# nianticlabs/mickey

Measured on AMD Instinct MI355X. Metric: image pairs/sec (540x720), higher is better.
Workload: dtype bf16

## Files before the change

include/mickey_hip_dev.h:

```cpp
#ifndef MICKEY_HIP_DEV_H
#define MICKEY_HIP_DEV_H

#ifdef __cplusplus
extern "C" {
#endif

int mk_gemm_set_tile(int mode);

int mk_attn_set_mode(int mode);

int mk_dev_mfma_sustained(float* scratch, int workgroups, int iters, int zero_operands, void* stream);

#ifdef __cplusplus
}
#endif
#endif
```

mickey_amd/_native.py:

```python
import ctypes
import os

import torch

from . import build as _build

MK_BF16, MK_F16, MK_F32 = 0, 1, 2
ACT_NONE, ACT_RELU, ACT_GELU = 0, 1, 2

_P, _I, _L, _F, _U = ctypes.c_void_p, ctypes.c_int, ctypes.c_longlong, ctypes.c_float, ctypes.c_ulonglong
_CODES = {"p": _P, "i": _I, "l": _L, "f": _F, "u": _U}

SIGNATURES = {
    "mk_version": ("i", ""),
    "mk_last_error": ("s", ""),
    "mk_preprocess_u8": ("i", "pliiipiip"),
    "mk_gemm": ("i", "pipippiiiiiiip"),
    "mk_gemm_grouped": ("i", "pilpilplpiliiiiiiip"),
    "mk_gemm_ls_residual": ("i", "pipipppiiiiip"),
    "mk_gemm_qkv": ("i", "pipippppiiiifip"),
    "mk_gemm_patch_embed": ("i", "pipipppiiiiip"),
    "mk_gemm_ls_residual_ln": ("i", "pipippppipppiiiiip"),
    "mk_gemm_patch_embed_ln": ("i", "pipipppppiiiiip"),
    "mk_cls_token_ln": ("i", "pppppiiiip"),
# ... 61 lines not shown
    "mk_dual_softmax": ("i", "ppppfifppppiiiip"),
    "mk_dual_softmax_split_work_floats": ("l", "iii"),
    "mk_dual_softmax_split": ("i", "ppppfifppppiiiip"),
    "mk_sinkhorn_work_floats": ("l", "iii"),
    "mk_sinkhorn": ("i", "ppppfippppiiiip"),
    "mk_dual_softmax_kf": ("i", "ppppfifppppiiiipip"),
    "mk_dual_softmax_split_kf": ("i", "ppppfifppppiiiipip"),
    "mk_sinkhorn_kf": ("i", "ppppfippppiiiipip"),
    "mk_mutual_nn": ("i", "ppppiiip"),
    "mk_dual_softmax_train_work_floats": ("l", "iiii"),
    "mk_dual_softmax_train": ("i", "ppppfppppppiiiiip"),
    "mk_dual_softmax_bwd_work_floats": ("l", "iiii"),
    "mk_dual_softmax_bwd": ("i", "ppppfpppppppppiiiiip"),
    "mk_exprace_topk_work_bytes": ("l", "iiil"),
    "mk_exprace_topk_state_bytes": ("l", "ii"),
    "mk_exprace_topk": ("i", "ppuupppppiiliip"),
    "mk_counter_add": ("i", "pup"),
    "mk_gather_backproject": ("i", "ppppppppppppiiiiip"),
    "mk_gather_backproject_kf": ("i", "ppppppppppppiiiiipip"),
    "mk_gather_backproject_bwd": ("i", "ppppppppppiiiiip"),
    "mk_ransac_hypotheses": ("i", "pppppuupfppppiiilp"),
    "mk_refine_pose": ("i", "pppppfiipppppppiiiip"),
    "mk_pose_finalize": ("i", "ppppip"),
    "mk_train_ransac_masks": ("i", "pppppuupfiipppiiilp"),
    "mk_reinforce_scatter": ("i", "ppppiiilp"),
    "mk_train_tail_fwd": ("i", "pppppppiiiifiifpppp"),
    "mk_train_tail_bwd": ("i", "pppppppiiiifiifppppppp"),
    "mk_train_aggregate_fwd": ("i", "pppiiififfppppp"),
    "mk_train_aggregate_bwd": ("i", "ppiiipp"),
}

DEV_SIGNATURES = {
    "mk_gemm_set_tile": ("i", "i"),
    "mk_attn_set_mode": ("i", "i"),
    "mk_dev_mfma_sustained": ("i", "piiip"),
}

_lib = None
_missing = set()


class MickeyHipError(RuntimeError):
    pass


def lib_path():
    return os.environ.get("MICKEY_HIP_LIB", _build.lib_path())


def load():
    global _lib
    if _lib is not None:
        return _lib
    path = lib_path()
    if not os.path.exists(path):
        raise MickeyHipError("libmickey_hip.so not found at %s -- build it with `python -m mickey_amd.build` "
                             "(mickey_amd has no CPU/ATen fallback)" % path)
    lib = ctypes.CDLL(path)
    for name, (res, args) in list(SIGNATURES.items()) + list(DEV_SIGNATURES.items()):
        try:
            fn = getattr(lib, name)
        except AttributeError:
            _missing.add(name)
            continue
        fn.restype = ctypes.c_char_p if res == "s" else _CODES[res]
        fn.argtypes = [_CODES[c] for c in args]
# ... 47 lines not shown
```

mickey_amd/csrc/mk_gemm.hip:

```cpp
#include "mk_gemm_common.hpp"

namespace mk {
namespace gemm {
namespace {

template <typename T, int AMODE, int WMF, bool SP = false>
__global__ __launch_bounds__(256, 1) void gemm_kernel(GemmParams p) {
  using V8 = typename Lp<T>::V8;
  constexpr int NWM = 2, NWN = 2;
  constexpr int NW = NWM * NWN, BM = NWM * WMF * 16, BN = NWN * 64;
  constexpr int AJ = BM / 8 / NW, WJ = BN / 8 / NW;
  constexpr int A_BYTES = BM * 128, STAGE_BYTES = (BM + BN) * 128;
  constexpr int NS = WMF == 2 ? 3 : 2;
  constexpr int PIECES = AJ + WJ;
  extern __shared__ __attribute__((aligned(16))) char smem[];

  const int tid = threadIdx.x;
  const int lane = tid & 63;
  const int wave = __builtin_amdgcn_readfirstlane(tid >> 6);
  const int wm = wave / NWN, wn = wave % NWN;
  const int g = blockIdx.y;
  const int ntm = (p.M + BM - 1) / BM, ntn = (p.N + BN - 1) / BN;
  const int nk = p.K / BK;
  const int fr = lane & 15, fg = lane >> 4;
// ... 63 lines not shown
#pragma unroll
        for (int mi = 0; mi < WMF; ++mi)
#pragma unroll
          for (int ni = 0; ni < 4; ++ni) acc[mi][ni] = Lp<T>::mma16(wf[ni], xf[mi], acc[mi][ni]);
      }
    }
  }
  epilogue<T, WMF>(p, acc, m0, n0, wm, wn, lane, g, lnp);
}

template <typename T, int AMODE, int WMF, bool SP = false>
int launch_small(const GemmParams& p, int groups, hipStream_t st) {
  constexpr int BM = 32 * WMF;
  constexpr int LDS = (WMF == 2 ? 3 : 2) * (BM + 128) * 128 + BM * 8;
  static bool attr_done = false;
  if (!attr_done) {
    hipError_t e = hipFuncSetAttribute((const void*)gemm_kernel<T, AMODE, WMF, SP>, hipFuncAttributeMaxDynamicSharedMemorySize, LDS);
    if (e != hipSuccess) {
      mk_set_error("gemm: cannot reserve %d B of LDS: %s", LDS, hipGetErrorString(e));
      return MK_ERR_LAUNCH;
    }
    attr_done = true;
  }
  const int ntm = (p.M + BM - 1) / BM, ntn = (p.N + 127) / 128;
  hipLaunchKernelGGL((gemm_kernel<T, AMODE, WMF, SP>), dim3(ntm * ntn, groups, 1), dim3(256), LDS, st, p);
  MK_CHECK_LAUNCH();
  return MK_OK;
}

int g_num_cus = 0;
int g_band_m = 0;
int g_half_rows = 1;
int g_schedule = 0;

template <int AMODE>
int launch(const GemmParams& p, int groups, int dtype, hipStream_t st) {
  const long long big_tiles = (long long)((p.M + 255) / 256) * ((p.N + 255) / 256) * groups;
  bool big = p.N >= 256 && big_tiles >= 192;
  const long long plmax = p.npass > 1 ? (long long)max(max(p.pl1[0], p.pl1[1]), max(p.pl2[0], p.pl2[1])) / 2 : 0;
  const bool k_ok = p.K >= 2 * BK && (long long)p.M * p.lda + plmax < (1ll << 31) && (long long)p.N * p.ldw < (1ll << 31) &&
                    (AMODE == A_DENSE || bordered_rows(p.M / (p.H * p.Wd), p.H, p.Wd) * (p.C1 > p.C2 ? p.C1 : p.C2) + plmax < (1ll << 31));
  const bool ln_fold = p.ln_stats || p.xh;
  if (dtype == MK_F32) {
    MK_CHECK_ARG(!ln_fold, "gemm: the folded-LayerNorm epilogues exist for 16-bit operands only");
    return launch_f32(p, groups, AMODE, st);
  }
  int sched = g_schedule;
  if (sched == 0) sched = (big && k_ok) ? 7 : 1;
  if (!k_ok) sched = 1;
  if (sched == 7) return launch_pp64(p, groups, dtype, AMODE, st, g_band_m);
  const long long small_tiles = (long long)((p.M + 127) / 128) * ((p.N + 127) / 128) * groups;
  const bool half_rows = g_schedule == 2 || (g_schedule != 1 && g_half_rows && small_tiles < 2 * num_cus() && p.M > 64);
  if (p.npass > 1)
    return half_rows ? launch_small<_Float16, AMODE, 2, true>(p, groups, st) : launch_small<_Float16, AMODE, 4, true>(p, groups, st);
  if (half_rows) return dtype == MK_BF16 ? launch_small<__bf16, AMODE, 2>(p, groups, st) : launch_small<_Float16, AMODE, 2>(p, groups, st);
  return dtype == MK_BF16 ? launch_small<__bf16, AMODE, 4>(p, groups, st) : launch_small<_Float16, AMODE, 4>(p, groups, st);
}

int check_common(const GemmParams& p, int dtype) {
  MK_CHECK_ARG(dtype == MK_BF16 || dtype == MK_F16 || dtype == MK_F32, "gemm: dtype must be MK_BF16, MK_F16 or MK_F32");
  MK_CHECK_ARG(p.M > 0 && p.N > 0 && p.K > 0, "gemm: empty problem M=%d N=%d K=%d", p.M, p.N, p.K);
  const int kt = dtype == MK_F32 ? KT<float> : BK;
  MK_CHECK_ARG(p.K % kt == 0, "gemm: K=%d must be a multiple of %d", p.K, kt);
  MK_CHECK_ARG(p.N % 4 == 0, "gemm: N=%d must be a multiple of 4", p.N);
  MK_CHECK_ARG(p.ldw % 8 == 0 && p.ldw >= p.K, "gemm: ldw=%d must be >= K and a multiple of 8", p.ldw);
  MK_CHECK_ARG(p.A && p.W, "gemm: null operand");
  return MK_OK;
}

}

int num_cus() {
  if (g_num_cus == 0) {
    int dev = 0, n = 0;
    if (hipGetDevice(&dev) != hipSuccess || hipDeviceGetAttribute(&n, hipDeviceAttributeMultiprocessorCount, dev) != hipSuccess || n <= 0)
      n = 256;
    g_num_cus = n;
  }
  return g_num_cus;
}

}
}

using namespace mk;
using namespace mk::gemm;

extern "C" {

int mk_gemm_set_tile(int mode) {
  if (mode >= 400 && mode < 464) {
    g_band_m = mode - 400;
    return MK_OK;
  }
  if (mode >= 464 && mode < 496) {
    g_band_m = -(mode - 464);
    return MK_OK;
  }
  if (mode == 500 || mode == 501) {
    g_half_rows = mode - 500;
    return MK_OK;
  }
  if (mode >= 600 && mode <= 602) {
    g_pp64_persist = mode - 600;
    return MK_OK;
  }
  MK_CHECK_ARG(mode == 0 || mode == 1 || mode == 2 || mode == 7,
               "mk_gemm_set_tile: unknown mode %d (0 automatic, 1 128x128, 2 64x128, 7 8-wave ping-pong)", mode);
  g_schedule = mode;
  return MK_OK;
}

int mk_gemm(const void* A, int lda, const void* W, int ldw, const float* bias, void* out, int ldc, int M, int N, int K,
            int act, int out_is_f32, int dtype, mk_stream_t stream) {
  GemmParams p = {};
  p.A = A; p.W = W; p.M = M; p.N = N; p.K = K; p.lda = lda; p.ldw = ldw;
  p.epi = MK_EPI_STORE; p.act = act; p.bias = bias; p.ldc = ldc;
  if (out_is_f32) p.out_f32 = (float*)out; else p.out_lp = out;
  if (int e = check_common(p, dtype)) return e;
  MK_CHECK_ARG(lda % 8 == 0 && lda >= K && ldc % 4 == 0 && ldc >= N && out, "mk_gemm: bad lda/ldc/out");
  return launch<A_DENSE>(p, 1, dtype, (hipStream_t)stream);
}

int mk_gemm_grouped(const void* A, int lda, long long strideA, const void* W, int ldw, long long strideW, const float* bias,
                    long long strideBias, void* out, int ldc, long long strideOut, int groups, int M, int N, int K, int act,
                    int out_is_f32, int dtype, mk_stream_t stream) {
  GemmParams p = {};
  p.A = A; p.W = W; p.M = M; p.N = N; p.K = K; p.lda = lda; p.ldw = ldw;
  p.strideA_g = strideA; p.strideW_g = strideW; p.strideBias_g = strideBias; p.strideOut_g = strideOut;
  p.epi = MK_EPI_STORE; p.act = act; p.bias = bias; p.ldc = ldc;
  if (out_is_f32) p.out_f32 = (float*)out; else p.out_lp = out;
  if (int e = check_common(p, dtype)) return e;
  MK_CHECK_ARG(groups > 0 && lda % 8 == 0 && lda >= K && ldc % 4 == 0 && ldc >= N && out, "mk_gemm_grouped: bad args");
  return launch<A_DENSE>(p, groups, dtype, (hipStream_t)stream);
}

int mk_gemm_ls_residual(const void* A, int lda, const void* W, int ldw, const float* bias, const float* gamma, float* x,
                        int ldx, int M, int N, int K, int dtype, mk_stream_t stream) {
  GemmParams p = {};
  p.A = A; p.W = W; p.M = M; p.N = N; p.K = K; p.lda = lda; p.ldw = ldw;
  p.epi = MK_EPI_LS_RESIDUAL; p.bias = bias; p.gamma = gamma; p.out_f32 = x; p.ldc = ldx;
  if (int e = check_common(p, dtype)) return e;
  MK_CHECK_ARG(bias && gamma && x && lda % 8 == 0 && lda >= K && ldx % 4 == 0 && ldx >= N, "mk_gemm_ls_residual: bad args");
  return launch<A_DENSE>(p, 1, dtype, (hipStream_t)stream);
// ... 194 lines not shown
```

mickey_amd/csrc/mk_gemm_common.hpp:

```cpp
#pragma once
#include "mk_common.hpp"

namespace mk {
namespace gemm {

constexpr int BK = 64;
template <typename T> constexpr int EPC = 16 / (int)sizeof(T);
template <typename T> constexpr int KT = 128 / (int)sizeof(T);

enum AMode { A_DENSE = 0, A_CONV3 = 1 };

struct GemmParams {
  const void* A;
  const void* A2;
  const void* W;
  int M, N, K, lda, ldw;
  long long strideA_g, strideA2_g, strideW_g;
  int H, Wd, C1, C2;
  int bord_out;
  unsigned pl1[2], pl2[2];
  int npass;
  float acc_scale;
  void* out_lo;
  float plane_scale;
  int* sat_flag;
  int epi;
  int act;
  const float* bias;
  const float* gamma;
  long long strideBias_g;
  float* out_f32;
  void* out_lp;
  int ldc;
  long long strideOut_g;
  const void* resid_lp;
  long long strideResid_g;
  void* q;
  void* k;
  void* vt;
  int ntok, ntok_pad, heads;
  float qscale;
  const float* pos;
  int npatch;
// ... 439 lines not shown
}

template <typename T, int WMF>
__device__ __forceinline__ void epilogue(const GemmParams& p, f32x4 (&acc)[WMF][4], int m0, int n0, int wm, int wn, int lane,
                                         int g, const float2* lnp = nullptr) {
  if (p.xh) {
    if (p.epi == MK_EPI_PATCH) epilogue_impl<T, WMF, MK_EPI_PATCH, MK_ACT_NONE, true, false, true>(p, acc, m0, n0, wm, wn, lane, g);
    else epilogue_impl<T, WMF, MK_EPI_LS_RESIDUAL, MK_ACT_NONE, true, false, true>(p, acc, m0, n0, wm, wn, lane, g);
    return;
  }
  if (p.ln_stats) {
    if (p.epi == MK_EPI_QKV) epilogue_impl<T, WMF, MK_EPI_QKV, MK_ACT_NONE, true, true>(p, acc, m0, n0, wm, wn, lane, g, lnp);
    else if (p.act == MK_ACT_GELU) epilogue_impl<T, WMF, MK_EPI_STORE, MK_ACT_GELU, true, true>(p, acc, m0, n0, wm, wn, lane, g, lnp);
    else epilogue_impl<T, WMF, MK_EPI_STORE, MK_ACT_NONE, true, true>(p, acc, m0, n0, wm, wn, lane, g, lnp);
    return;
  }
  switch (p.epi) {
    case MK_EPI_LS_RESIDUAL: epilogue_impl<T, WMF, MK_EPI_LS_RESIDUAL, MK_ACT_NONE, true>(p, acc, m0, n0, wm, wn, lane, g); break;
    case MK_EPI_QKV: epilogue_impl<T, WMF, MK_EPI_QKV, MK_ACT_NONE, true>(p, acc, m0, n0, wm, wn, lane, g); break;
    case MK_EPI_PATCH: epilogue_impl<T, WMF, MK_EPI_PATCH, MK_ACT_NONE, true>(p, acc, m0, n0, wm, wn, lane, g); break;
    default:
      if (!p.bias) {
        if (p.act == MK_ACT_RELU) epilogue_impl<T, WMF, MK_EPI_STORE, MK_ACT_RELU, false>(p, acc, m0, n0, wm, wn, lane, g);
        else if (p.act == MK_ACT_GELU) epilogue_impl<T, WMF, MK_EPI_STORE, MK_ACT_GELU, false>(p, acc, m0, n0, wm, wn, lane, g);
        else epilogue_impl<T, WMF, MK_EPI_STORE, MK_ACT_NONE, false>(p, acc, m0, n0, wm, wn, lane, g);
      } else {
        if (p.act == MK_ACT_RELU) epilogue_impl<T, WMF, MK_EPI_STORE, MK_ACT_RELU, true>(p, acc, m0, n0, wm, wn, lane, g);
        else if (p.act == MK_ACT_GELU) epilogue_impl<T, WMF, MK_EPI_STORE, MK_ACT_GELU, true>(p, acc, m0, n0, wm, wn, lane, g);
        else epilogue_impl<T, WMF, MK_EPI_STORE, MK_ACT_NONE, true>(p, acc, m0, n0, wm, wn, lane, g);
      }
  }
}

template <typename T, int EPI, int ACT, bool HAS_BIAS, bool LN = false, bool SPLIT = false, bool FIN = false, bool CONV = false>
__device__ __forceinline__ void epilogue_lds_impl(const GemmParams& p, f32x4 (&acc)[8][4], char* wl0, char* wl1, int m0, int n0, int wm,
                                                  int wn, int lane, int g, const float2* lnp = nullptr) {
  using V4 = typename Lp<T>::V4;
  using V8 = typename Lp<T>::V8;
  const int fr = lane & 15, fg = lane >> 4;
  const float* bias = HAS_BIAS ? p.bias + (long long)g * p.strideBias_g : nullptr;
  const int nw = n0 + wn * 64;
  const int mw = m0 + wm * 128;
  int img0 = 0, tok0 = 0;
  if (EPI == MK_EPI_QKV) {
    img0 = mw / p.ntok;
    tok0 = mw - img0 * p.ntok;
  }
  auto img_tok = [&](int r, int& img, int& tok) {
    if (p.ntok >= 128) {
      const int t = tok0 + r;
      const bool wrap = t >= p.ntok;
      img = img0 + (wrap ? 1 : 0);
      tok = wrap ? t - p.ntok : t;
    } else {
      const int m = mw + r;
      img = m / p.ntok;
      tok = m - img * p.ntok;
    }
  };
  f32x4 bv[4], cs[4];
#pragma unroll
  for (int ni = 0; ni < 4; ++ni) {
    const int n = nw + fg * 4 + ni * 16;
    bv[ni] = (HAS_BIAS && n < p.N) ? *(const f32x4*)(bias + n) : f32x4{0.f, 0.f, 0.f, 0.f};
    cs[ni] = (LN && n < p.N) ? *(const f32x4*)(p.ln_colsum + n) : f32x4{0.f, 0.f, 0.f, 0.f};
  }
  float2 prm[8];
#pragma unroll
  for (int mi = 0; mi < 8; ++mi) prm[mi] = LN ? lnp[wm * 128 + mi * 16 + fr] : make_float2(1.f, 0.f);
  const bool lp_out = EPI == MK_EPI_QKV || (EPI == MK_EPI_STORE && !p.out_f32 && !p.out_lo);
  if (lp_out) {
    int which = 0, head = 0;
    if (EPI == MK_EPI_QKV) {
      const int D = p.heads * 64;
      which = nw / D;
      head = (nw - which * D) >> 6;
      if (which == 2) {
#pragma unroll
        for (int mi = 0; mi < 8; ++mi) {
          const int m = mw + mi * 16 + fr;
          if (m >= p.M) continue;
          int img, tok;
          img_tok(mi * 16 + fr, img, tok);
          const long long hb = (long long)img * p.heads + head;
#pragma unroll
          for (int ni = 0; ni < 4; ++ni) {
            const f32x4 v = LN ? acc[mi][ni] * prm[mi].x + (cs[ni] * prm[mi].y + bv[ni]) : acc[mi][ni] + bv[ni];
            T* dst = (T*)p.vt + (hb * 64 + ni * 16 + fg * 4) * p.ntok_pad + vperm(tok);
#pragma unroll
            for (int e = 0; e < 4; ++e) dst[(long long)e * p.ntok_pad] = to_lp<T>(v[e]);
          }
        }
        return;
      }
    }
    const int rr = lane >> 3, c = lane & 7;
    const int n = nw + c * 8;
    const bool bord = CONV && p.bord_out;
    BorderedRow bw;
    if (bord) bw.init(mw + rr, p.H, p.Wd);
#pragma unroll
    for (int h = 0; h < 2; ++h) {
#pragma unroll
      for (int mq = 0; mq < 4; ++mq) {
        const int mi = h * 4 + mq;
        const int r = mi * 16 + fr;
        char* wrow = (mq < 2 ? wl0 : wl1) + ((mq & 1) * 16 + fr) * 128;
        const long long rrow = (CONV && p.resid_lp) ? bordered_row(min(mw + r, p.M - 1), p.H, p.Wd) : 0;
#pragma unroll
        for (int ni = 0; ni < 4; ++ni) {
          f32x4 v = acc[mi][ni];
          if (LN) v = v * prm[mi].x + (cs[ni] * prm[mi].y + bv[ni]);
          else if (HAS_BIAS) v += bv[ni];
          if (EPI == MK_EPI_QKV) {
            if (which == 0) { const float qs = p.qscale; _Pragma("unroll") for (int e = 0; e < 4; ++e) v[e] *= qs; }
          } else {
            if (CONV && p.resid_lp) {
              const int m = mw + r, n2 = nw + fg * 4 + ni * 16;
              if (m < p.M && n2 < p.N) {
                const V4 rs = *(const V4*)((const T*)p.resid_lp + (long long)g * p.strideResid_g + rrow * p.ldc + n2);
#pragma unroll
                for (int e = 0; e < 4; ++e) v[e] += (float)rs[e];
              }
            }
            if (ACT == MK_ACT_RELU) {
#pragma unroll
              for (int e = 0; e < 4; ++e) v[e] = fmaxf(v[e], 0.f);
            } else if (ACT == MK_ACT_GELU) {
              v = gelu_erf4(v);
            }
          }
          V4 o;
#pragma unroll
          for (int e = 0; e < 4; ++e) o[e] = to_lp<T>(v[e]);
          const int cc = ni * 2 + (fg >> 1);
          *(V4*)(wrow + ((cc ^ (fr & 7)) << 4) + (fg & 1) * 8) = o;
        }
      }
#pragma unroll
      for (int i8 = 0; i8 < 8; ++i8) {
        const int it = h * 8 + i8;
        const int r = it * 8 + rr;
        const int m = mw + r;
        const V8 val = *(const V8*)((i8 < 4 ? wl0 : wl1) + ((i8 & 3) * 8 + rr) * 128 + ((c ^ (rr & 7)) << 4));
        const int extra = bord ? bw.extra : 0;
        if (bord) bw.step(8, p.H, p.Wd);
        if (m >= p.M || n >= p.N) continue;
        T* dst;
        if (EPI == MK_EPI_QKV) {
          int img, tok;
          img_tok(r, img, tok);
          dst = (T*)(which == 0 ? p.q : p.k) + (((long long)img * p.heads + head) * p.ntok_pad + tok) * 64 + c * 8;
        } else {
          dst = (T*)p.out_lp + (long long)g * p.strideOut_g + ((long long)m + extra) * p.ldc + n;
        }
        if (n + 8 <= p.N) {
          *(V8*)dst = val;
        } else {
          V4 lo;
#pragma unroll
          for (int e = 0; e < 4; ++e) lo[e] = val[e];
          *(V4*)dst = lo;
        }
      }
    }
  } else {
    const int rr = lane >> 4, c = lane & 15;
    const int n = nw + c * 4;
    f32x4 gm = f32x4{0.f, 0.f, 0.f, 0.f};
    if (EPI == MK_EPI_LS_RESIDUAL && n < p.N) gm = *(const f32x4*)(p.gamma + n);
    f32x4 bvd = f32x4{0.f, 0.f, 0.f, 0.f};
    if (SPLIT && HAS_BIAS && n < p.N) bvd = *(const f32x4*)(bias + n);
    f32x4 xr[2][SPLIT ? 1 : 16];
// ... 116 lines not shown
          x += gm * val;
          if (SPLIT) x -= ((const float*)lnp)[wm * 128 + half * 64 + r];
          if (!SPLIT || fin) {
            if (ok) *(f32x4*)(p.out_f32 + (long long)m * p.ldc + n) = x;
          } else {
            if constexpr (sizeof(T) == 2) emit_row(m, nullptr, nullptr, x, ok, soff_b(half, it));
            else emit_row(m, plane_row(p.xh, half, it) + lane_off_st, plane_row(p.xl, half, it) + lane_off_st, x, ok);
          }
        } else if (EPI == MK_EPI_PATCH) {
          const int mc = ok ? m : 0;
          const int img = mc / p.npatch, tok = mc - img * p.npatch;
          const long long xrow = (long long)img * (p.npatch + 1) + 1 + tok;
          f32x4 x = val;
          if (ok) x += *(const f32x4*)(p.pos + (long long)(1 + tok) * p.N + n);
          if (SPLIT) emit_row(xrow, (T*)p.xh + xrow * p.ldxs + n, (T*)p.xl + xrow * p.ldxs + n, x, ok);
          else if (ok) *(f32x4*)(p.out_f32 + xrow * p.ldc + n) = x;
        } else if (EPI == MK_EPI_STORE && p.out_lo) {
          const float ps = p.plane_scale;
          f16x4 oh, ol;
#pragma unroll
          for (int e = 0; e < 4; ++e) {
            const float sv = sat16(val[e] * ps, p.sat_flag);
            oh[e] = (_Float16)sv;
            ol[e] = (_Float16)(sv - (float)oh[e]);
          }
          const long long o = (long long)g * p.strideOut_g + ((long long)m + extraf) * p.ldc + n;
          *(f16x4*)((_Float16*)p.out_lp + o) = oh;
          *(f16x4*)((_Float16*)p.out_lo + o) = ol;
        } else {
          *(f32x4*)(p.out_f32 + (long long)g * p.strideOut_g + ((long long)m + extraf) * p.ldc + n) = val;
        }
      }
    };
    if (SPLIT && !FIN && EPI == MK_EPI_LS_RESIDUAL) {
      preload(0, 0, 16);
      stageq(0, 0);
      drain(0, 0, 8);
      preload(1, 0, 8);
      stageq(0, 1);
      drain(0, 8, 16);
      preload(1, 8, 16);
      stageq(1, 0);
      drain(1, 0, 8);
      stageq(1, 1);
      drain(1, 8, 16);
    } else {
      preload(0);
      stageq(0, 0);
      drain(0, 0, 8);
      stageq(0, 1);
      preload(1);
      drain(0, 8, 16);
      stageq(1, 0);
      drain(1, 0, 8);
      stageq(1, 1);
      drain(1, 8, 16);
    }
  }
}

template <typename T, int KIND, bool CONV = false, int BN = 256>
__device__ __forceinline__ void epilogue_lds(const GemmParams& p, f32x4 (&acc)[8][4], char* wl0, char* wl1, int m0, int n0, int wm,
                                             int wn, int lane, int g, const float2* lnp = nullptr) {
  if constexpr (KIND == 2 || KIND == 3) {
    const bool interior = m0 + 256 <= p.M && n0 + BN <= p.N;
    if (KIND == 3) {
      if (interior) epilogue_lds_impl<T, MK_EPI_LS_RESIDUAL, MK_ACT_NONE, true, false, true, true>(p, acc, wl0, wl1, m0, n0, wm, wn, lane, g, lnp);
// ... 3 lines not shown
      else epilogue_impl<T, 8, MK_EPI_PATCH, MK_ACT_NONE, true, false, true>(p, acc, m0, n0, wm, wn, lane, g);
    } else {
      if (interior) epilogue_lds_impl<T, MK_EPI_LS_RESIDUAL, MK_ACT_NONE, true, false, true, false>(p, acc, wl0, wl1, m0, n0, wm, wn, lane, g, lnp);
      else epilogue_impl<T, 8, MK_EPI_LS_RESIDUAL, MK_ACT_NONE, true, false, true>(p, acc, m0, n0, wm, wn, lane, g);
    }
  } else if constexpr (KIND == 1) {
#if defined(MK_LN_ABL) && MK_LN_ABL == 2
    constexpr bool LNE = false;
#else
    constexpr bool LNE = true;
#endif
    if (p.epi == MK_EPI_QKV) epilogue_lds_impl<T, MK_EPI_QKV, MK_ACT_NONE, true, LNE>(p, acc, wl0, wl1, m0, n0, wm, wn, lane, g, lnp);
    else if (p.act == MK_ACT_GELU) epilogue_lds_impl<T, MK_EPI_STORE, MK_ACT_GELU, true, LNE>(p, acc, wl0, wl1, m0, n0, wm, wn, lane, g, lnp);
    else epilogue_lds_impl<T, MK_EPI_STORE, MK_ACT_NONE, true, LNE>(p, acc, wl0, wl1, m0, n0, wm, wn, lane, g, lnp);
  } else {
    switch (CONV ? MK_EPI_STORE : p.epi) {
      case MK_EPI_LS_RESIDUAL: epilogue_lds_impl<T, MK_EPI_LS_RESIDUAL, MK_ACT_NONE, true>(p, acc, wl0, wl1, m0, n0, wm, wn, lane, g); break;
      case MK_EPI_QKV: epilogue_lds_impl<T, MK_EPI_QKV, MK_ACT_NONE, true>(p, acc, wl0, wl1, m0, n0, wm, wn, lane, g); break;
      case MK_EPI_PATCH: epilogue_lds_impl<T, MK_EPI_PATCH, MK_ACT_NONE, true>(p, acc, wl0, wl1, m0, n0, wm, wn, lane, g); break;
      default:
        if (!p.bias) {
          if (p.act == MK_ACT_RELU) epilogue_lds_impl<T, MK_EPI_STORE, MK_ACT_RELU, false, false, false, false, CONV>(p, acc, wl0, wl1, m0, n0, wm, wn, lane, g);
          else if (!CONV && p.act == MK_ACT_GELU) epilogue_lds_impl<T, MK_EPI_STORE, MK_ACT_GELU, false>(p, acc, wl0, wl1, m0, n0, wm, wn, lane, g);
          else epilogue_lds_impl<T, MK_EPI_STORE, MK_ACT_NONE, false, false, false, false, CONV>(p, acc, wl0, wl1, m0, n0, wm, wn, lane, g);
        } else {
          if (p.act == MK_ACT_RELU) epilogue_lds_impl<T, MK_EPI_STORE, MK_ACT_RELU, true, false, false, false, CONV>(p, acc, wl0, wl1, m0, n0, wm, wn, lane, g);
          else if (!CONV && p.act == MK_ACT_GELU) epilogue_lds_impl<T, MK_EPI_STORE, MK_ACT_GELU, true>(p, acc, wl0, wl1, m0, n0, wm, wn, lane, g);
          else epilogue_lds_impl<T, MK_EPI_STORE, MK_ACT_NONE, true, false, false, false, CONV>(p, acc, wl0, wl1, m0, n0, wm, wn, lane, g);
        }
    }
  }
}

__device__ __forceinline__ void pp_tile_coords(int id, int ntm, int ntn, int PP_GM, int& tm, int& tn) {
  if (PP_GM < 0) {
    const int ng = -PP_GM;
    const int grp = id / (ntm * ng);
    const int rem = id - grp * (ntm * ng);
    const int gn = min(ng, ntn - grp * ng);
    tm = rem / gn;
    tn = grp * ng + rem - tm * gn;
    return;
  }
  const int band = id / (PP_GM * ntn);
  const int rem = id - band * (PP_GM * ntn);
  const int gm = min(PP_GM, ntm - band * PP_GM);
  tm = band * PP_GM + rem % gm;
  tn = rem / gm;
}

int num_cus();
extern int g_pp64_persist;
int launch_pp64(const GemmParams& p, int groups, int dtype, int amode, hipStream_t st, int band_m);
int launch_f32(const GemmParams& p, int groups, int amode, hipStream_t st);

}
}
```

mickey_amd/csrc/mk_gemm_pp64.hip:

```cpp
#include <type_traits>

#include "mk_gemm_common.hpp"

namespace mk {
namespace gemm {
int g_pp64_persist = 2;
namespace {

template <typename T, int AMODE, int KIND, bool PERSIST = false, bool SP = false, bool SP2 = false>
__global__ __launch_bounds__(512, 2) void gemm_pp64_kernel(GemmParams p, int band_m) {
  static_assert(!SP2 || SP, "SP2 is a form of the split-operand kernel");
  static_assert(!PERSIST || AMODE == A_DENSE, "the persistent tile loop is built for dense operands");
  static_assert(!SP || (KIND == 0 && !PERSIST && sizeof(T) == 2), "split operands: plain epilogues, one tile per workgroup");
  constexpr int BKA = SP ? BK / 2 : BK;
  using V8 = typename Lp<T>::V8;
  constexpr int WMF = 8, BM = 256, BN = 256;
  constexpr int A_BYTES = BM * 128, STAGE_BYTES = (BM + BN) * 128;
  constexpr int LN_STAGE_OFF = 2 * STAGE_BYTES + 256 * 8;
  extern __shared__ __attribute__((aligned(16))) char smem[];

  const int tid0 = threadIdx.x;
  const int wave = __builtin_amdgcn_readfirstlane(tid0 >> 6);
  int lane = tid0 & 63, tid = tid0;
  auto refresh_lane = [&]() {
    if constexpr (PERSIST) {
      asm volatile("v_mbcnt_lo_u32_b32 %0, -1, 0\n\tv_mbcnt_hi_u32_b32 %0, -1, %0" : "=v"(lane));
      tid = wave * 64 + lane;
    }
  };
  const int wm = wave >> 2, wn = wave & 3;
  const int g = blockIdx.y;
  const int ntm = (p.M + BM - 1) / BM, ntn = (p.N + BN - 1) / BN;
  const int nk = p.K / BK;

  const T* A = (const T*)p.A + (long long)g * p.strideA_g;
  const T* A2 = p.A2 ? (const T*)p.A2 + (long long)g * p.strideA2_g : nullptr;
  const T* W = (const T*)p.W + (long long)g * p.strideW_g;
  int srow = lane >> 3, sp = lane & 7;
  const int ntiles = ntm * ntn;
  auto tile_origin = [&](int id, int& mm, int& nn) {
    int tm, tn;
    pp_tile_coords(xcd_remap(id, ntiles), ntm, ntn, band_m, tm, tn);
    mm = tm * BM;
    nn = tn * BN;
  };
  int bid = blockIdx.x;
  int m0, n0;
  tile_origin(bid, m0, n0);
  unsigned woff[4], aoff[4], aoff2[4];
  auto set_woff = [&](int nn0) {
#pragma unroll
    for (int j = 0; j < 4; ++j) {
      const int rw = (wave * 4 + j) * 8 + srow;
      int n = nn0 + rw;
      n = n < p.N ? n : p.N - 1;
      woff[j] = ((unsigned)n * (unsigned)p.ldw + swz8(rw, sp) * 8) * (unsigned)sizeof(T);
    }
  };
  auto set_aoff = [&](int mm0) {
#pragma unroll
    for (int j = 0; j < 4; ++j) {
      const int ra = wm * 128 + (wn * 4 + j) * 8 + srow;
      int m = mm0 + ra;
      m = m < p.M ? m : p.M - 1;
      const int c = swz8(ra, sp);
      const unsigned cc = SP ? (unsigned)(c & 3) : (unsigned)c;
      const bool lo = SP && (c >> 2) != 0;
      const unsigned pb1 = !SP ? 0u : (lo ? p.pl1[1] : p.pl1[0]), pb2 = !SP ? 0u : (lo ? p.pl2[1] : p.pl2[0]);
      if (AMODE == A_DENSE) {
        aoff[j] = ((unsigned)m * (unsigned)p.lda + cc * 8) * (unsigned)sizeof(T) + pb1;
        aoff2[j] = 0;
      } else {
        const unsigned br = (unsigned)bordered_row(m, p.H, p.Wd);
        aoff[j] = (br * (unsigned)p.C1 + cc * 8) * (unsigned)sizeof(T) + pb1;
        aoff2[j] = (br * (unsigned)p.C2 + cc * 8) * (unsigned)sizeof(T) + pb2;
      }
    }
  };
  set_woff(n0);
  set_aoff(m0);
  auto dma_w1 = [&](int s, int j) {
    glds16_sv(W + s * BK, woff[j], smem + (s & 1) * STAGE_BYTES + A_BYTES + (wave * 4 + j) * 1024);
  };
  const int ntap = A2 ? 10 : 9;
  const T* cbase = AMODE == A_DENSE ? A : A - (long long)(p.Wd + 2) * p.C1;
  int cleft = p.C1, ctap = 0;
  auto conv_advance = [&]() {
    cleft -= BKA;
    const bool wrap = cleft == 0;
    ctap += wrap ? 1 : 0;
    const int ty = (ctap * 11) >> 5, tx = ctap - 3 * ty;
    const T* tapbase = ctap < 9 ? A + (long long)((ty - 1) * (p.Wd + 1) + tx - 1) * p.C1 : A2;
    cbase = wrap ? tapbase : cbase + BKA;
    cleft = wrap ? (ctap < 9 ? p.C1 : p.C2) : cleft;
  };
  auto dma_a1 = [&](int s, int j) {
    char* dst = smem + (s & 1) * STAGE_BYTES + (wm * 16 + wn * 4 + j) * 1024;
    if (AMODE == A_DENSE) {
      glds16_sv(A + s * BKA, aoff[j], dst);
    } else {
      glds16_sv(cbase, ctap < 9 ? aoff[j] : aoff2[j], dst);
    }
  };
  auto dma_w = [&](int s) {
#pragma unroll
    for (int j = 0; j < 4; ++j) dma_w1(s, j);
  };
  auto dma_a = [&](int s) {
#pragma unroll
    for (int j = 0; j < 4; ++j) dma_a1(s, j);
    if (AMODE != A_DENSE) conv_advance();
  };

  int fr = lane & 15, fg = lane >> 4;
  auto derive_lane = [&]() {
    srow = lane >> 3;
    sp = lane & 7;
    fr = lane & 15;
    fg = lane >> 4;
  };
  auto load_w = [&](V8* wf, int par, int h) {
    const char* sW = smem + par * STAGE_BYTES + A_BYTES;
#pragma unroll
    for (int i = 0; i < 4; ++i) {
      const int rw = wn * 64 + i * 16 + fr;
      wf[i] = *(const V8*)(sW + rw * 128 + swz8(rw, h * 4 + fg) * 16);
    }
  };
  auto load_x = [&](V8* xf, int par, int h) {
    const char* sA = smem + par * STAGE_BYTES;
#pragma unroll
    for (int i = 0; i < WMF; ++i) {
      const int rx = wm * 128 + i * 16 + fr;
      xf[i] = *(const V8*)(sA + rx * 128 + swz8(rx, h * 4 + fg) * 16);
    }
  };
  auto load_frags = [&](V8* wf, V8* xf, int par, int h) {
    load_w(wf, par, h);
    load_x(xf, par, h);
  };
  f32x4 acc[WMF][4];
  auto zero_acc = [&]() {
#pragma unroll
    for (int i = 0; i < WMF; ++i)
#pragma unroll
      for (int j = 0; j < 4; ++j) acc[i][j] = f32x4{0.f, 0.f, 0.f, 0.f};
  };
  if constexpr (!PERSIST) zero_acc();
  auto mfma32 = [&](const V8* wf, const V8* xf, auto dma, int s, auto first) {
    constexpr bool DMA = decltype(dma)::value;
    constexpr bool FIRST = decltype(first)::value;
    __builtin_amdgcn_s_setprio(1);
    __builtin_amdgcn_sched_barrier(0);
#pragma unroll
    for (int q = 0; q < 32; ++q) {
      const int mi = q >> 2, ni = q & 3;
      acc[mi][ni] = Lp<T>::mma16(wf[ni], xf[mi], FIRST ? f32x4{0.f, 0.f, 0.f, 0.f} : acc[mi][ni]);
      if (DMA && (q & 7) == 3) {
        __builtin_amdgcn_sched_barrier(0);
        dma_a1(s, q >> 3);
        __builtin_amdgcn_sched_barrier(0);
      }
    }
    __builtin_amdgcn_sched_barrier(0);
    __builtin_amdgcn_s_setprio(0);
    if (DMA && AMODE != A_DENSE) conv_advance();
  };
  auto bar = [&]() {
    asm volatile("s_waitcnt lgkmcnt(0)" ::: "memory");
    __builtin_amdgcn_s_barrier();
  };
  using Yes = std::integral_constant<bool, true>;
  using No = std::integral_constant<bool, false>;
  V8 wf[4], xf[WMF];
  V8 wfl[SP ? 4 : 1];
  auto stage0 = [&](int kt, auto next1, auto next2, int sw, int sa, auto first) {
    if constexpr (SP && SP2) {
      bar();
      load_frags(wf, xf, kt & 1, 0);
      if constexpr (decltype(next1)::value) dma_w(sw);
      bar();
      mfma32(wf, xf, No{}, 0, first);
      bar();
      load_w(wf, kt & 1, 1);
      bar();
      mfma32(wf, xf, next2, sa, No{});
      if constexpr (decltype(next2)::value)
        asm volatile("s_waitcnt vmcnt(4)" ::: "memory");
      else
        asm volatile("s_waitcnt vmcnt(0)" ::: "memory");
      return;
    }
    if constexpr (SP) {
// ... 142 lines not shown
        kt0 = 2;
      }
      for (int kt = kt0; kt < nk - 2; ++kt) stage0(kt, Yes{}, Yes{}, kt + 1, kt + 2, No{});
      if constexpr (PERSIST) {
        set_aoff(m1);
        stage0(nk - 2, Yes{}, Yes{}, nk - 1, 0, No{});
        set_woff(n1);
        stage0(nk - 1, Yes{}, No{}, 0, 0, No{});
      } else {
        stage0(nk - 2, Yes{}, No{}, nk - 1, 0, No{});
        stage0(nk - 1, No{}, No{}, 0, 0, No{});
      }
      bar();
    } else {
      bar();
      if constexpr (PERSIST) {
        stage1(0, Yes{}, Yes{}, 1, 2, Yes{});
        first_stage_done();
        stage1(1, Yes{}, Yes{}, 2, 3, No{});
        second_stage_done();
        kt0 = 2;
      }
      for (int kt = kt0; kt < nk - 2; ++kt) stage1(kt, Yes{}, Yes{}, kt + 1, kt + 2, No{});
      if constexpr (PERSIST) {
        set_aoff(m1);
        stage1(nk - 2, Yes{}, Yes{}, nk - 1, 0, No{});
        set_woff(n1);
        stage1(nk - 1, Yes{}, No{}, 0, 0, No{});
      } else {
        stage1(nk - 2, Yes{}, No{}, nk - 1, 0, No{});
        stage1(nk - 1, No{}, No{}, 0, 0, No{});
      }
    }
    char* wl0 = smem + STAGE_BYTES + wave * 4096;
    refresh_lane();
    epilogue_lds<T, KIND, AMODE == A_CONV3>(p, acc, wl0, wl0 + A_BYTES, m0, n0, wm, wn, lane, g, (const float2*)(smem + 2 * STAGE_BYTES));
    if (!(PERSIST && has_next)) break;
    bid = nbid;
    m0 = m1;
    n0 = n1;
    asm volatile("" : "+s"(m0), "+s"(n0));
    refresh_lane();
    if (ln_fast) LnRowDma16::issue<0>(p, m0, wave, lane, smem + LN_STAGE_OFF);
    if constexpr (PRODUCER) shl.issue(p, m0, tid, 256);
  }
}

template <typename T, int AMODE, int KIND, bool PERSIST, bool SP = false, bool SP2 = false>
int launch_k2(const GemmParams& p, int groups, hipStream_t st, int band_m, int grid) {
  constexpr int LDS = 2 * 512 * 128 + 256 * 8 + (PERSIST && KIND == 1 ? 16384 : 0);
  static bool attr_done = false;
  if (!attr_done) {
    hipError_t e = hipFuncSetAttribute((const void*)gemm_pp64_kernel<T, AMODE, KIND, PERSIST, SP, SP2>, hipFuncAttributeMaxDynamicSharedMemorySize, LDS);
    if (e != hipSuccess) {
      mk_set_error("gemm: cannot reserve %d B of LDS: %s", LDS, hipGetErrorString(e));
      return MK_ERR_LAUNCH;
    }
    attr_done = true;
  }
  hipLaunchKernelGGL((gemm_pp64_kernel<T, AMODE, KIND, PERSIST, SP, SP2>), dim3(grid, groups, 1), dim3(512), LDS, st, p, band_m);
  MK_CHECK_LAUNCH();
  return MK_OK;
}

template <typename T, int AMODE, int KIND>
int launch_k(const GemmParams& p, int groups, hipStream_t st, int band_m) {
  const int ntm = (p.M + 255) / 256, ntn = (p.N + 255) / 256;
  if (band_m == 0) band_m = (AMODE == A_DENSE && ntn <= 4) ? -4 : 8;
  if constexpr (KIND == 0 && sizeof(T) == 2 && std::is_same<T, _Float16>::value) {
    if (p.npass == 2) {
      if constexpr (AMODE == A_CONV3) return launch_k2<T, AMODE, 0, false, true, true>(p, groups, st, band_m, ntm * ntn);
    }
    if (p.npass > 1) return launch_k2<T, AMODE, 0, false, true>(p, groups, st, band_m, ntm * ntn);
  }
  if constexpr (AMODE == A_DENSE && KIND != 0) {
    const int nk = p.K / BK, grid = num_cus() & ~7;
    const bool ok = groups == 1 && p.npass <= 1 && (nk & 1) == 0 && nk >= 4 && grid >= 8 && ntm * ntn > grid &&
                    !(KIND == 1 && p.ln_stats && p.ln_nslot != 16);
    if (g_pp64_persist != 1 && ok && !(g_pp64_persist == 2 && KIND == 1)) return launch_k2<T, AMODE, KIND, true>(p, groups, st, band_m, grid);
  }
  return launch_k2<T, AMODE, KIND, false>(p, groups, st, band_m, ntm * ntn);
}

template <typename T>
int launch_dense(const GemmParams& p, int groups, hipStream_t st, int band_m) {
  if (p.xh && p.epi == MK_EPI_LS_RESIDUAL && p.out_f32) return launch_k<T, A_DENSE, 3>(p, groups, st, band_m);
  if (p.xh) return launch_k<T, A_DENSE, 2>(p, groups, st, band_m);
  if (p.ln_stats) return launch_k<T, A_DENSE, 1>(p, groups, st, band_m);
  return launch_k<T, A_DENSE, 0>(p, groups, st, band_m);
}

}

int launch_pp64(const GemmParams& p, int groups, int dtype, int amode, hipStream_t st, int band_m) {
  if (amode == A_DENSE) return dtype == MK_BF16 ? launch_dense<__bf16>(p, groups, st, band_m) : launch_dense<_Float16>(p, groups, st, band_m);
  return dtype == MK_BF16 ? launch_k<__bf16, A_CONV3, 0>(p, groups, st, band_m) : launch_k<_Float16, A_CONV3, 0>(p, groups, st, band_m);
}

}
}
```

mickey_amd/ops.py:

```python

import numpy as np
import torch


from ._native import ACT_GELU, ACT_NONE, ACT_RELU, call, dtype_code, ptr, query, stream

LOG2E = 1.4426950408889634


def _chk(t, dtype=None):
    assert t.is_cuda and t.is_contiguous(), "expected a contiguous device tensor"
    if dtype is not None:
        assert t.dtype == dtype, "expected %s, got %s" % (dtype, t.dtype)
    return t


def preprocess_u8(frames, H, W, out=None):
    assert frames.is_cuda and frames.dtype == torch.uint8 and frames.dim() == 4 and frames.shape[3] == 3 and frames.is_contiguous()
    n, Hs, Ws, _ = frames.shape
    if out is None:
        out = torch.empty((n, 3, H, W), device=frames.device, dtype=torch.float32)
    call("mk_preprocess_u8", ptr(frames), Hs * Ws * 3, n, Hs, Ws, ptr(out), H, W, stream())
    return out


def gemm_set_tile(mode):
    call("mk_gemm_set_tile", int(mode))


def gemm(a, w, bias=None, act=ACT_NONE, out_f32=False, out=None, lda=None, K=None):
    M = a.shape[0]
    lda = a.shape[1] if lda is None else lda
    N, ldw = w.shape
    K = min(lda, ldw) if K is None else K
    if out is None:
        out = torch.empty((M, N), device=a.device, dtype=torch.float32 if out_f32 else a.dtype)
    call("mk_gemm", ptr(a), lda, ptr(w), ldw, ptr(bias), ptr(out), out.stride(0), M, N, K, act,
         int(out.dtype == torch.float32), dtype_code(a.dtype), stream())
    return out


def gemm_grouped(a, w, bias, out, groups, M, N, K, lda, ldw, ldc, stride_a, stride_w, stride_bias, stride_out, act=ACT_NONE):
    call("mk_gemm_grouped", ptr(a), lda, stride_a, ptr(w), ldw, stride_w, ptr(bias), stride_bias, ptr(out), ldc, stride_out,
         groups, M, N, K, act, int(out.dtype == torch.float32), dtype_code(a.dtype), stream())
    return out


def gemm_ls_residual(a, w, bias, gamma, x):
    M, K = a.shape
    N = w.shape[0]
    call("mk_gemm_ls_residual", ptr(a), a.stride(0), ptr(w), w.stride(0), ptr(bias), ptr(gamma), ptr(x), x.stride(0), M, N, K,
         dtype_code(a.dtype), stream())
    return x


def gemm_qkv(a, w, bias, q, k, vt, nimg, ntok, ntok_pad, heads):
    qscale = (64.0 ** -0.5) * LOG2E
    call("mk_gemm_qkv", ptr(a), a.stride(0), ptr(w), w.stride(0), ptr(bias), ptr(q), ptr(k), ptr(vt), nimg, ntok, ntok_pad,
         heads, qscale, dtype_code(a.dtype), stream())

# ... 882 lines not shown
```

Measured before the change: 271.2.

## Add narrow 256x128 and 256x64 ping-pong tiles for conv3x3 GEMMs

Adds narrow-N variants of the 8-wave ping-pong GEMM kernel for 3x3 convolutions with 128 or 64 output channels. These replace the 256x256 tile, which leaves half or three quarters of its columns idle when N is 128 or 64. The new variants use less LDS and a different wave-to-fragment mapping, and the 64-wide one allows higher occupancy. They are picked by default when the tile count is large. A debug query reports which schedule was chosen last. The risk is that each MFMA sees less reuse of the A operand, and the new epilogue paths are more complex.

After: 271.8, median of 6. Within noise of the previous version (+0.2%).

```diff
diff --git a/include/mickey_hip_dev.h b/include/mickey_hip_dev.h
--- a/include/mickey_hip_dev.h
+++ b/include/mickey_hip_dev.h
@@ -7,6 +7,8 @@
 
 int mk_gemm_set_tile(int mode);
 
+int mk_gemm_last_schedule(void);
+
 int mk_attn_set_mode(int mode);
 
 int mk_dev_mfma_sustained(float* scratch, int workgroups, int iters, int zero_operands, void* stream);
diff --git a/mickey_amd/_native.py b/mickey_amd/_native.py
--- a/mickey_amd/_native.py
+++ b/mickey_amd/_native.py
@@ -117,6 +117,7 @@
 
 DEV_SIGNATURES = {
     "mk_gemm_set_tile": ("i", "i"),
+    "mk_gemm_last_schedule": ("i", ""),
     "mk_attn_set_mode": ("i", "i"),
     "mk_dev_mfma_sustained": ("i", "piiip"),
 }
diff --git a/mickey_amd/csrc/mk_gemm.hip b/mickey_amd/csrc/mk_gemm.hip
--- a/mickey_amd/csrc/mk_gemm.hip
+++ b/mickey_amd/csrc/mk_gemm.hip
@@ -119,25 +119,36 @@
 int g_band_m = 0;
 int g_half_rows = 1;
 int g_schedule = 0;
+int g_narrow = 0;
+int g_last = 0;
+constexpr int PP_MIN_TILES = 192;
 
 template <int AMODE>
 int launch(const GemmParams& p, int groups, int dtype, hipStream_t st) {
   const long long big_tiles = (long long)((p.M + 255) / 256) * ((p.N + 255) / 256) * groups;
-  bool big = p.N >= 256 && big_tiles >= 192;
+  bool big = p.N >= 256 && big_tiles >= PP_MIN_TILES;
   const long long plmax = p.npass > 1 ? (long long)max(max(p.pl1[0], p.pl1[1]), max(p.pl2[0], p.pl2[1])) / 2 : 0;
   const bool k_ok = p.K >= 2 * BK && (long long)p.M * p.lda + plmax < (1ll << 31) && (long long)p.N * p.ldw < (1ll << 31) &&
                     (AMODE == A_DENSE || bordered_rows(p.M / (p.H * p.Wd), p.H, p.Wd) * (p.C1 > p.C2 ? p.C1 : p.C2) + plmax < (1ll << 31));
   const bool ln_fold = p.ln_stats || p.xh;
   if (dtype == MK_F32) {
     MK_CHECK_ARG(!ln_fold, "gemm: the folded-LayerNorm epilogues exist for 16-bit operands only");
+    g_last = 32;
     return launch_f32(p, groups, AMODE, st);
+  }
+  if (AMODE == A_CONV3 && (p.N == 128 || p.N == 64) && p.npass <= 1 && k_ok &&
+      (g_narrow == 2 || (g_narrow == 0 && g_schedule == 0 && big_tiles >= PP_MIN_TILES))) {
+    g_last = p.N == 128 ? 71 : 72;
+    return launch_pp64_narrow(p, groups, dtype, st, g_band_m);
   }
   int sched = g_schedule;
   if (sched == 0) sched = (big && k_ok) ? 7 : 1;
   if (!k_ok) sched = 1;
+  g_last = sched == 7 ? 7 : 1;
   if (sched == 7) return launch_pp64(p, groups, dtype, AMODE, st, g_band_m);
   const long long small_tiles = (long long)((p.M + 127) / 128) * ((p.N + 127) / 128) * groups;
   const bool half_rows = g_schedule == 2 || (g_schedule != 1 && g_half_rows && small_tiles < 2 * num_cus() && p.M > 64);
+  if (half_rows) g_last = 2;
   if (p.npass > 1)
     return half_rows ? launch_small<_Float16, AMODE, 2, true>(p, groups, st) : launch_small<_Float16, AMODE, 4, true>(p, groups, st);
   if (half_rows) return dtype == MK_BF16 ? launch_small<__bf16, AMODE, 2>(p, groups, st) : launch_small<_Float16, AMODE, 2>(p, groups, st);
@@ -192,11 +203,17 @@
     g_pp64_persist = mode - 600;
     return MK_OK;
   }
+  if (mode >= 700 && mode <= 702) {
+    g_narrow = mode - 700;
+    return MK_OK;
+  }
   MK_CHECK_ARG(mode == 0 || mode == 1 || mode == 2 || mode == 7,
                "mk_gemm_set_tile: unknown mode %d (0 automatic, 1 128x128, 2 64x128, 7 8-wave ping-pong)", mode);
   g_schedule = mode;
   return MK_OK;
 }
+
+int mk_gemm_last_schedule(void) { return g_last; }
 
 int mk_gemm(const void* A, int lda, const void* W, int ldw, const float* bias, void* out, int ldc, int M, int N, int K,
             int act, int out_is_f32, int dtype, mk_stream_t stream) {
diff --git a/mickey_amd/csrc/mk_gemm_common.hpp b/mickey_amd/csrc/mk_gemm_common.hpp
--- a/mickey_amd/csrc/mk_gemm_common.hpp
+++ b/mickey_amd/csrc/mk_gemm_common.hpp
@@ -8,7 +8,7 @@
 template <typename T> constexpr int EPC = 16 / (int)sizeof(T);
 template <typename T> constexpr int KT = 128 / (int)sizeof(T);
 
-enum AMode { A_DENSE = 0, A_CONV3 = 1 };
+enum AMode { A_DENSE = 0, A_CONV3 = 1, A_CONV3_N128 = 2, A_CONV3_N64 = 3 };
 
 struct GemmParams {
   const void* A;
@@ -514,15 +514,16 @@
   }
 }
 
-template <typename T, int EPI, int ACT, bool HAS_BIAS, bool LN = false, bool SPLIT = false, bool FIN = false, bool CONV = false>
-__device__ __forceinline__ void epilogue_lds_impl(const GemmParams& p, f32x4 (&acc)[8][4], char* wl0, char* wl1, int m0, int n0, int wm,
+template <typename T, int EPI, int ACT, bool HAS_BIAS, bool LN = false, bool SPLIT = false, bool FIN = false, bool CONV = false, int WMF = 8>
+__device__ __forceinline__ void epilogue_lds_impl(const GemmParams& p, f32x4 (&acc)[WMF][4], char* wl0, char* wl1, int m0, int n0, int wm,
                                                   int wn, int lane, int g, const float2* lnp = nullptr) {
+  static_assert(WMF == 8 || ((WMF == 4 || WMF == 2) && CONV && EPI == MK_EPI_STORE && !LN && !SPLIT), "narrow blocks: plain conv epilogues");
   using V4 = typename Lp<T>::V4;
   using V8 = typename Lp<T>::V8;
   const int fr = lane & 15, fg = lane >> 4;
   const float* bias = HAS_BIAS ? p.bias + (long long)g * p.strideBias_g : nullptr;
   const int nw = n0 + wn * 64;
-  const int mw = m0 + wm * 128;
+  const int mw = m0 + wm * (WMF * 16);
   int img0 = 0, tok0 = 0;
   if (EPI == MK_EPI_QKV) {
     img0 = mw / p.ntok;
@@ -547,9 +548,9 @@
     bv[ni] = (HAS_BIAS && n < p.N) ? *(const f32x4*)(bias + n) : f32x4{0.f, 0.f, 0.f, 0.f};
     cs[ni] = (LN && n < p.N) ? *(const f32x4*)(p.ln_colsum + n) : f32x4{0.f, 0.f, 0.f, 0.f};
   }
-  float2 prm[8];
-#pragma unroll
-  for (int mi = 0; mi < 8; ++mi) prm[mi] = LN ? lnp[wm * 128 + mi * 16 + fr] : make_float2(1.f, 0.f);
+  float2 prm[WMF];
+#pragma unroll
+  for (int mi = 0; mi < WMF; ++mi) prm[mi] = LN ? lnp[wm * 128 + mi * 16 + fr] : make_float2(1.f, 0.f);
   const bool lp_out = EPI == MK_EPI_QKV || (EPI == MK_EPI_STORE && !p.out_f32 && !p.out_lo);
   if (lp_out) {
     int which = 0, head = 0;
@@ -559,7 +560,7 @@
       head = (nw - which * D) >> 6;
       if (which == 2) {
 #pragma unroll
-        for (int mi = 0; mi < 8; ++mi) {
+        for (int mi = 0; mi < WMF; ++mi) {
           const int m = mw + mi * 16 + fr;
           if (m >= p.M) continue;
           int img, tok;
@@ -581,10 +582,11 @@
     const bool bord = CONV && p.bord_out;
     BorderedRow bw;
     if (bord) bw.init(mw + rr, p.H, p.Wd);
-#pragma unroll
-    for (int h = 0; h < 2; ++h) {
-#pragma unroll
-      for (int mq = 0; mq < 4; ++mq) {
+    constexpr int MQ = WMF < 4 ? WMF : 4;
+#pragma unroll
+    for (int h = 0; h < WMF / MQ; ++h) {
+#pragma unroll
+      for (int mq = 0; mq < MQ; ++mq) {
         const int mi = h * 4 + mq;
         const int r = mi * 16 + fr;
         char* wrow = (mq < 2 ? wl0 : wl1) + ((mq & 1) * 16 + fr) * 128;
@@ -620,7 +622,7 @@
         }
       }
 #pragma unroll
-      for (int i8 = 0; i8 < 8; ++i8) {
+      for (int i8 = 0; i8 < 2 * MQ; ++i8) {
         const int it = h * 8 + i8;
         const int r = it * 8 + rr;
         const int m = mw + r;
@@ -803,7 +805,15 @@
         }
       }
     };
-    if (SPLIT && !FIN && EPI == MK_EPI_LS_RESIDUAL) {
+    if constexpr (WMF == 2) {
+      stageq(0, 0);
+      drain(0, 0, 8);
+    } else if constexpr (WMF == 4) {
+      stageq(0, 0);
+      drain(0, 0, 8);
+      stageq(0, 1);
+      drain(0, 8, 16);
+    } else if (SPLIT && !FIN && EPI == MK_EPI_LS_RESIDUAL) {
       preload(0, 0, 16);
       stageq(0, 0);
       drain(0, 0, 8);
@@ -873,6 +883,19 @@
   }
 }
 
+template <typename T, int BN>
+__device__ __forceinline__ void epilogue_lds_narrow(const GemmParams& p, f32x4 (&acc)[BN / 32][4], char* wl0, char* wl1, int m0, int n0,
+                                                    int wm, int wn, int lane, int g) {
+  constexpr int WMF = BN / 32;
+  if (!p.bias) {
+    if (p.act == MK_ACT_RELU) epilogue_lds_impl<T, MK_EPI_STORE, MK_ACT_RELU, false, false, false, false, true, WMF>(p, acc, wl0, wl1, m0, n0, wm, wn, lane, g);
+    else epilogue_lds_impl<T, MK_EPI_STORE, MK_ACT_NONE, false, false, false, false, true, WMF>(p, acc, wl0, wl1, m0, n0, wm, wn, lane, g);
+  } else {
+    if (p.act == MK_ACT_RELU) epilogue_lds_impl<T, MK_EPI_STORE, MK_ACT_RELU, true, false, false, false, true, WMF>(p, acc, wl0, wl1, m0, n0, wm, wn, lane, g);
+    else epilogue_lds_impl<T, MK_EPI_STORE, MK_ACT_NONE, true, false, false, false, true, WMF>(p, acc, wl0, wl1, m0, n0, wm, wn, lane, g);
+  }
+}
+
 __device__ __forceinline__ void pp_tile_coords(int id, int ntm, int ntn, int PP_GM, int& tm, int& tn) {
   if (PP_GM < 0) {
     const int ng = -PP_GM;
@@ -893,6 +916,7 @@
 int num_cus();
 extern int g_pp64_persist;
 int launch_pp64(const GemmParams& p, int groups, int dtype, int amode, hipStream_t st, int band_m);
+int launch_pp64_narrow(const GemmParams& p, int groups, int dtype, hipStream_t st, int band_m);
 int launch_f32(const GemmParams& p, int groups, int amode, hipStream_t st);
 
 }
diff --git a/mickey_amd/csrc/mk_gemm_pp64.hip b/mickey_amd/csrc/mk_gemm_pp64.hip
--- a/mickey_amd/csrc/mk_gemm_pp64.hip
+++ b/mickey_amd/csrc/mk_gemm_pp64.hip
@@ -8,13 +8,17 @@
 namespace {
 
 template <typename T, int AMODE, int KIND, bool PERSIST = false, bool SP = false, bool SP2 = false>
-__global__ __launch_bounds__(512, 2) void gemm_pp64_kernel(GemmParams p, int band_m) {
+__global__ __launch_bounds__(512, AMODE == A_CONV3_N64 ? 4 : 2) void gemm_pp64_kernel(GemmParams p, int band_m) {
+  constexpr int BN = AMODE == A_CONV3_N128 ? 128 : AMODE == A_CONV3_N64 ? 64 : 256;
   static_assert(!SP2 || SP, "SP2 is a form of the split-operand kernel");
   static_assert(!PERSIST || AMODE == A_DENSE, "the persistent tile loop is built for dense operands");
   static_assert(!SP || (KIND == 0 && !PERSIST && sizeof(T) == 2), "split operands: plain epilogues, one tile per workgroup");
+  static_assert(BN == 256 || (KIND == 0 && !PERSIST && !SP), "the narrow tiles carry the plain convs only");
   constexpr int BKA = SP ? BK / 2 : BK;
   using V8 = typename Lp<T>::V8;
-  constexpr int WMF = 8, BM = 256, BN = 256;
+  constexpr int BM = 256, WMF = BN / 32;
+  constexpr int WJ = BN / 64;
+  constexpr int NMF = WMF * 4;
   constexpr int A_BYTES = BM * 128, STAGE_BYTES = (BM + BN) * 128;
   constexpr int LN_STAGE_OFF = 2 * STAGE_BYTES + 256 * 8;
   extern __shared__ __attribute__((aligned(16))) char smem[];
@@ -47,11 +51,11 @@
   int bid = blockIdx.x;
   int m0, n0;
   tile_origin(bid, m0, n0);
-  unsigned woff[4], aoff[4], aoff2[4];
+  unsigned woff[WJ], aoff[4], aoff2[4];
   auto set_woff = [&](int nn0) {
 #pragma unroll
-    for (int j = 0; j < 4; ++j) {
-      const int rw = (wave * 4 + j) * 8 + srow;
+    for (int j = 0; j < WJ; ++j) {
+      const int rw = (wave * WJ + j) * 8 + srow;
       int n = nn0 + rw;
       n = n < p.N ? n : p.N - 1;
       woff[j] = ((unsigned)n * (unsigned)p.ldw + swz8(rw, sp) * 8) * (unsigned)sizeof(T);
@@ -80,7 +84,7 @@
   set_woff(n0);
   set_aoff(m0);
   auto dma_w1 = [&](int s, int j) {
-    glds16_sv(W + s * BK, woff[j], smem + (s & 1) * STAGE_BYTES + A_BYTES + (wave * 4 + j) * 1024);
+    glds16_sv(W + s * BK, woff[j], smem + (s & 1) * STAGE_BYTES + A_BYTES + (wave * WJ + j) * 1024);
   };
   const int ntap = A2 ? 10 : 9;
   const T* cbase = AMODE == A_DENSE ? A : A - (long long)(p.Wd + 2) * p.C1;
@@ -104,7 +108,7 @@
   };
   auto dma_w = [&](int s) {
 #pragma unroll
-    for (int j = 0; j < 4; ++j) dma_w1(s, j);
+    for (int j = 0; j < WJ; ++j) dma_w1(s, j);
   };
   auto dma_a = [&](int s) {
 #pragma unroll
@@ -119,11 +123,21 @@
     fr = lane & 15;
     fg = lane >> 4;
   };
+  auto wcol0 = [&]() {
+    if constexpr (BN == 256) return wn * 64;
+    else if constexpr (BN == 128) return (wn & 1) * 64;
+    else return 0;
+  };
+  auto xrow0 = [&]() {
+    if constexpr (BN == 256) return wm * 128;
+    else if constexpr (BN == 128) return wm * 128 + (wn >> 1) * 64;
+    else return wave * 32;
+  };
   auto load_w = [&](V8* wf, int par, int h) {
     const char* sW = smem + par * STAGE_BYTES + A_BYTES;
 #pragma unroll
     for (int i = 0; i < 4; ++i) {
-      const int rw = wn * 64 + i * 16 + fr;
+      const int rw = wcol0() + i * 16 + fr;
       wf[i] = *(const V8*)(sW + rw * 128 + swz8(rw, h * 4 + fg) * 16);
     }
   };
@@ -131,7 +145,7 @@
     const char* sA = smem + par * STAGE_BYTES;
 #pragma unroll
     for (int i = 0; i < WMF; ++i) {
-      const int rx = wm * 128 + i * 16 + fr;
+      const int rx = xrow0() + i * 16 + fr;
       xf[i] = *(const V8*)(sA + rx * 128 + swz8(rx, h * 4 + fg) * 16);
     }
   };
@@ -150,15 +164,16 @@
   auto mfma32 = [&](const V8* wf, const V8* xf, auto dma, int s, auto first) {
     constexpr bool DMA = decltype(dma)::value;
     constexpr bool FIRST = decltype(first)::value;
+    constexpr int PER = NMF / 4;
     __builtin_amdgcn_s_setprio(1);
     __builtin_amdgcn_sched_barrier(0);
 #pragma unroll
-    for (int q = 0; q < 32; ++q) {
+    for (int q = 0; q < NMF; ++q) {
       const int mi = q >> 2, ni = q & 3;
       acc[mi][ni] = Lp<T>::mma16(wf[ni], xf[mi], FIRST ? f32x4{0.f, 0.f, 0.f, 0.f} : acc[mi][ni]);
-      if (DMA && (q & 7) == 3) {
+      if (DMA && q % PER == (PER - 1) / 2) {
         __builtin_amdgcn_sched_barrier(0);
-        dma_a1(s, q >> 3);
+        dma_a1(s, q / PER);
         __builtin_amdgcn_sched_barrier(0);
       }
     }
@@ -367,9 +382,14 @@
         stage1(nk - 1, No{}, No{}, 0, 0, No{});
       }
     }
-    char* wl0 = smem + STAGE_BYTES + wave * 4096;
-    refresh_lane();
-    epilogue_lds<T, KIND, AMODE == A_CONV3>(p, acc, wl0, wl0 + A_BYTES, m0, n0, wm, wn, lane, g, (const float2*)(smem + 2 * STAGE_BYTES));
+    if constexpr (BN != 256) {
+      char* wl = smem + wave * 8192;
+      epilogue_lds_narrow<T, BN>(p, acc, wl, wl + 4096, m0, n0, xrow0() / (16 * WMF), wcol0() / 64, lane, g);
+    } else {
+      char* wl0 = smem + STAGE_BYTES + wave * 4096;
+      refresh_lane();
+      epilogue_lds<T, KIND, AMODE == A_CONV3>(p, acc, wl0, wl0 + A_BYTES, m0, n0, wm, wn, lane, g, (const float2*)(smem + 2 * STAGE_BYTES));
+    }
     if (!(PERSIST && has_next)) break;
     bid = nbid;
     m0 = m1;
@@ -383,7 +403,8 @@
 
 template <typename T, int AMODE, int KIND, bool PERSIST, bool SP = false, bool SP2 = false>
 int launch_k2(const GemmParams& p, int groups, hipStream_t st, int band_m, int grid) {
-  constexpr int LDS = 2 * 512 * 128 + 256 * 8 + (PERSIST && KIND == 1 ? 16384 : 0);
+  constexpr int BN = AMODE == A_CONV3_N128 ? 128 : AMODE == A_CONV3_N64 ? 64 : 256;
+  constexpr int LDS = BN != 256 ? 2 * (256 + BN) * 128 : 2 * 512 * 128 + 256 * 8 + (PERSIST && KIND == 1 ? 16384 : 0);
   static bool attr_done = false;
   if (!attr_done) {
     hipError_t e = hipFuncSetAttribute((const void*)gemm_pp64_kernel<T, AMODE, KIND, PERSIST, SP, SP2>, hipFuncAttributeMaxDynamicSharedMemorySize, LDS);
@@ -396,6 +417,14 @@
   hipLaunchKernelGGL((gemm_pp64_kernel<T, AMODE, KIND, PERSIST, SP, SP2>), dim3(grid, groups, 1), dim3(512), LDS, st, p, band_m);
   MK_CHECK_LAUNCH();
   return MK_OK;
+}
+
+template <typename T>
+int launch_narrow(const GemmParams& p, int groups, hipStream_t st, int band_m) {
+  const int ntm = (p.M + 255) / 256;
+  if (band_m == 0) band_m = 8;
+  if (p.N == 128) return launch_k2<T, A_CONV3_N128, 0, false>(p, groups, st, band_m, ntm);
+  return launch_k2<T, A_CONV3_N64, 0, false>(p, groups, st, band_m, ntm);
 }
 
 template <typename T, int AMODE, int KIND>
@@ -432,5 +461,9 @@
   return dtype == MK_BF16 ? launch_k<__bf16, A_CONV3, 0>(p, groups, st, band_m) : launch_k<_Float16, A_CONV3, 0>(p, groups, st, band_m);
 }
 
-}
-}
+int launch_pp64_narrow(const GemmParams& p, int groups, int dtype, hipStream_t st, int band_m) {
+  return dtype == MK_BF16 ? launch_narrow<__bf16>(p, groups, st, band_m) : launch_narrow<_Float16>(p, groups, st, band_m);
+}
+
+}
+}
diff --git a/mickey_amd/ops.py b/mickey_amd/ops.py
--- a/mickey_amd/ops.py
+++ b/mickey_amd/ops.py
@@ -26,6 +26,10 @@
 
 def gemm_set_tile(mode):
     call("mk_gemm_set_tile", int(mode))
+
+
+def gemm_last_schedule():
+    return int(query("mk_gemm_last_schedule"))
 
 
 def gemm(a, w, bias=None, act=ACT_NONE, out_f32=False, out=None, lda=None, K=None):
```
